# FrancescoI/torchrecsys

Hardware: AMD Instinct MI355X
Metric: training interactions/sec (pos+neg) (higher is better)
Workload: dtype f32; 1 GPU; c4 per-GPU shard: net_type='fm', 10M users x 1M items, 125M-interaction shard of 1B, dim=128, per-GPU batch 32768 (global 262144 at 8 GPUs); global_batch=32768, per_gpu_batch=32768, rng=device (Feistel epoch shuffle + Philox4x32-10 negative sampler)

## Files before the change

### torchrecsys_amd/csrc/api.cpp

```cpp
#include "trs_common.h"

#include <string.h>

static thread_local char g_err[512] = "";

void trs_set_error(const char* fmt, ...) {
  va_list ap;
  va_start(ap, fmt);
  vsnprintf(g_err, sizeof(g_err), fmt, ap);
  va_end(ap);
}

extern "C" const char* trs_last_error(void) { return g_err; }

#include <mutex>
#include <stdlib.h>

namespace {
struct Knob {
  const char* name;
  int64_t TrsTuning::*wide;
  int TrsTuning::*narrow;
  int64_t unset;
};
const Knob KNOBS[] = {
    {"GRID_CAP", &TrsTuning::grid_cap, nullptr, 256 * 16},
    {"PASS_GRID_CAP", &TrsTuning::pass_grid_cap, nullptr, 4096},
    {"PRESORT_GRID_CAP", &TrsTuning::presort_grid_cap, nullptr, 512},
    {"K1_ITERS", nullptr, &TrsTuning::k1_iters, 0},
    {"PASS_ITERS", nullptr, &TrsTuning::pass_iters, 0},
    {"PASS_NT", nullptr, &TrsTuning::pass_nt, -1},
    {"K1_NT", nullptr, &TrsTuning::k1_nt, -1},
    {"K1_WGS_PER_CU", nullptr, &TrsTuning::k1_wgs_per_cu, 2},
    {"GEMM32_NO_GLDS", nullptr, &TrsTuning::gemm32_no_glds, 0},
    {"GEMM16_TN_WIDE", nullptr, &TrsTuning::gemm16_tn_wide, -1},
    {"GEMM16_TILE", nullptr, &TrsTuning::gemm16_tile, 0},
    {"GEMM16_NO_GLDS", nullptr, &TrsTuning::gemm16_no_glds, 0},
    {"BN_FINAL_TWO_SWEEPS", nullptr, &TrsTuning::bn_final_two_sweeps, 0},
};
TrsTuning g_tuning;
std::once_flag g_tuning_once;
void knob_store(const Knob& k, int64_t v) {
  if (k.wide) g_tuning.*(k.wide) = v;
  else g_tuning.*(k.narrow) = (int)v;
}
}

TrsTuning& trs_tuning() {
  std::call_once(g_tuning_once, [] {
    for (const Knob& k : KNOBS) {
      char name[64];
      snprintf(name, sizeof(name), "TRS_%s", k.name);
      const char* e = getenv(name);
      knob_store(k, (e && *e) ? atoll(e) : k.unset);
    }
  });
  return g_tuning;
}

extern "C" int trs_tuning_set(const char* name, int64_t value, int32_t unset) {
  TRS_REQUIRE(name != nullptr, "trs_tuning_set: NULL name");
  (void)trs_tuning();
  for (const Knob& k : KNOBS)
    if (strcmp(k.name, name) == 0) {
      knob_store(k, unset ? k.unset : value);
      return TRS_OK;
    }
  trs_set_error("trs_tuning_set: unknown knob %s", name);
  return TRS_E_ARG;
}

extern "C" int trs_abi_version(void) { return TRS_ABI_VERSION; }

extern "C" int trs_check_device(void) {
  int dev = -1;
  if (hipGetDevice(&dev) != hipSuccess) {
    trs_set_error("trs_check_device: no HIP device");
    (void)hipGetLastError();
    return TRS_E_DEVICE;
  }
  hipDeviceProp_t p;
  if (hipGetDeviceProperties(&p, dev) != hipSuccess) {
    trs_set_error("trs_check_device: hipGetDeviceProperties failed");
    (void)hipGetLastError();
    return TRS_E_DEVICE;
  }
  if (strncmp(p.gcnArchName, "gfx950", 6) != 0) {
    trs_set_error("trs_check_device: device %d is %s, this library is built for gfx950 only", dev, p.gcnArchName);
    return TRS_E_DEVICE;
  }
  return TRS_OK;
}

extern "C" int trs_events_create(int32_t n, void** handles_out) {
  TRS_REQUIRE(n >= 0 && (n == 0 || handles_out), "trs_events_create: bad arguments");
  for (int32_t i = 0; i < n; ++i) {
    hipEvent_t e;
    if (hipEventCreate(&e) != hipSuccess) {
      trs_set_error("trs_events_create: hipEventCreate failed");
      (void)hipGetLastError();
      return TRS_E_LAUNCH;
    }
    handles_out[i] = (void*)e;
  }
  return TRS_OK;
}

extern "C" int trs_events_destroy(int32_t n, void** handles) {
  for (int32_t i = 0; i < n; ++i)
    if (handles && handles[i]) (void)hipEventDestroy((hipEvent_t)handles[i]);
  return TRS_OK;
}

extern "C" int trs_events_elapsed_ms(void* start, void* stop, float* ms_out) {
  TRS_REQUIRE(start && stop && ms_out, "trs_events_elapsed_ms: NULL argument");
  if (hipEventElapsedTime(ms_out, (hipEvent_t)start, (hipEvent_t)stop) != hipSuccess) {
    trs_set_error("trs_events_elapsed_ms: events not complete (synchronise the stream first)");
    (void)hipGetLastError();
    return TRS_E_LAUNCH;
  }
  return TRS_OK;
}
```

### torchrecsys_amd/csrc/presort.hip

```cpp
#include <cstring>

#include "score_kernels.h"
#include "opt_rows.h"

#ifndef K2_WAVES
#define K2_WAVES 4
#endif
namespace trs {

struct RefPayload {
  uint32_t tw;
};

struct EpochArgs {
  const int2* sui;
  const int32_t* neg_static;
  int64_t N;
  uint64_t shuffle_key;
  int hb;
  uint64_t sample_seed;
  int64_t first_pos;
  int64_t n_pos;
  int64_t batch;
  int64_t n_users, n_items;
  int item_bits;
  int32_t* user;
  int32_t* pos;
  int32_t* neg;
  void* keys;
  RefPayload* vals;
  int32_t* err;
  TrsSampler S;
};

template <typename KeyT, int SRC>
__global__ __launch_bounds__(TRS_BLOCK) void epoch_refs_kernel(const EpochArgs a) {
  const int64_t stride = (int64_t)gridDim.x * TRS_BLOCK;
  KeyT* keys = reinterpret_cast<KeyT*>(a.keys);
  for (int64_t q = (int64_t)blockIdx.x * TRS_BLOCK + threadIdx.x; q < a.n_pos; q += stride) {
    int64_t u, i, j;
    if (SRC != 0) {
      const int64_t p = trs_feistel_perm(a.first_pos + q, a.N * a.S.k_neg, a.shuffle_key, a.hb) % a.N;
      const int2 ui = a.sui[p];
      u = ui.x;
      i = ui.y;
      j = SRC == 2 ? (int64_t)a.neg_static[p]
                   : ((uint64_t)u < (uint64_t)a.n_users && (uint64_t)i < (uint64_t)a.n_items
                          ? trs_sample_neg_opt(a.sample_seed, (uint64_t)(a.first_pos + q), u, i, a.n_items, a.S)
                          : 0);
    } else {
      u = a.user[q];
      i = a.pos[q];
      j = a.neg[q];
    }
    bool ok = true;
    if ((uint64_t)u >= (uint64_t)a.n_users) { ok = false; u = 0; }
    if ((uint64_t)i >= (uint64_t)a.n_items) { ok = false; i = 0; }
    if ((uint64_t)j >= (uint64_t)a.n_items) { ok = false; j = 0; }
    if (!ok && a.err) atomicOr(a.err, 1);
    if (SRC != 0 || !ok) {
      a.user[q] = (int32_t)u;
      a.pos[q] = (int32_t)i;
      a.neg[q] = (int32_t)j;
    }
    if (keys) {
      keys[2 * q] = (KeyT)i;
      keys[2 * q + 1] = (KeyT)j;
    }
  }
}

struct FlagArgs {
  const int2* sui;
  const int32_t* neg_static;
  int64_t N;
  uint64_t shuffle_key;
  int hb;
  uint64_t sample_seed;
  int64_t first_pos, batch;
  int64_t n_users, n_items;
  int32_t *user, *pos, *neg;
  uint8_t* uflags;
  uint8_t* iflags;
  int32_t* err;
  int log2_bits;
  int item_hash, user_hash;
  int what_first, what_end;
  int32_t* nflag;
  int ord_off, ord_cap;
};

constexpr int FLAG_THREADS = 1024;

__device__ __forceinline__ uint32_t flag_bit(int32_t row, int hashed, int log2_bits) {
  return hashed ? ((uint32_t)row * 2654435761u) >> (32 - log2_bits) : (uint32_t)row;
}

constexpr int FLAG_U = 8;
constexpr int FLAG_ROUNDS = 8;
constexpr int FLAG_MAX_GROUPS = 4;

template <int NG>
__global__ __launch_bounds__(FLAG_THREADS) void batch_flags_kernel(const FlagArgs a) {
  extern __shared__ uint32_t bm[];
  const int words = 1 << (a.log2_bits - 5);
  const int64_t q0 = (int64_t)blockIdx.x * a.batch;
  const int B = (int)a.batch;
  const int lb = a.log2_bits;
  uint16_t* iflags16 = reinterpret_cast<uint16_t*>(a.iflags);
  constexpr int STEP = FLAG_THREADS * FLAG_U;
  uint64_t anyf[NG];
#pragma unroll
  for (int g = 0; g < NG; ++g) anyf[g] = 0;
  for (int what = a.what_first; what < a.what_end; ++what) {
    const int hashed = what == 0 ? a.item_hash : a.user_hash;
    const int32_t* ida = what == 0 ? a.pos : a.user;
    uint64_t lat0[NG], lat1[NG];
#pragma unroll
    for (int g = 0; g < NG; ++g) lat0[g] = lat1[g] = 0;
    for (int w = threadIdx.x; w < words; w += FLAG_THREADS) bm[w] = 0u;
    __syncthreads();
#pragma unroll
    for (int g = 0; g < NG; ++g) {
#pragma unroll 1
    for (int rr = 0; rr < FLAG_ROUNDS && (g * FLAG_ROUNDS + rr) * STEP < B; ++rr) {
      const int rd = g * FLAG_ROUNDS + rr;
      const int t0 = threadIdx.x + rd * STEP;
      uint32_t b0[FLAG_U], b1[FLAG_U];
#pragma unroll
      for (int k = 0; k < FLAG_U; ++k) {
        const int t = t0 + k * FLAG_THREADS;
        const int64_t q = q0 + (t < B ? t : 0);
        b0[k] = flag_bit(ida[q], hashed, lb);
        b1[k] = what == 0 ? flag_bit(a.neg[q], hashed, lb) : 0u;
      }
#pragma unroll
      for (int k = 0; k < FLAG_U; ++k) {
        if (t0 + k * FLAG_THREADS < B) {
          const uint32_t o0 = atomicOr(&bm[b0[k] >> 5], 1u << (b0[k] & 31));
          lat0[g] |= (uint64_t)((o0 >> (b0[k] & 31)) & 1u) << (rr * FLAG_U + k);
          if (what == 0) {
            const uint32_t o1 = atomicOr(&bm[b1[k] >> 5], 1u << (b1[k] & 31));
            lat1[g] |= (uint64_t)((o1 >> (b1[k] & 31)) & 1u) << (rr * FLAG_U + k);
          }
        }
      }
    }
    }
    __syncthreads();
    for (int w = threadIdx.x; w < words; w += FLAG_THREADS) bm[w] = 0u;
    __syncthreads();
#pragma unroll
    for (int g = 0; g < NG; ++g) {
      for (uint64_t m = lat0[g]; m; m &= m - 1) {
        const int bit = __ffsll((unsigned long long)m) - 1;
        const int64_t q = q0 + threadIdx.x + (int64_t)(g * FLAG_ROUNDS + bit / FLAG_U) * STEP + (bit % FLAG_U) * FLAG_THREADS;
        const uint32_t b = flag_bit(ida[q], hashed, lb);
        atomicOr(&bm[b >> 5], 1u << (b & 31));
      }
      for (uint64_t m = lat1[g]; m; m &= m - 1) {
        const int bit = __ffsll((unsigned long long)m) - 1;
        const int64_t q = q0 + threadIdx.x + (int64_t)(g * FLAG_ROUNDS + bit / FLAG_U) * STEP + (bit % FLAG_U) * FLAG_THREADS;
        const uint32_t b = flag_bit(a.neg[q], hashed, lb);
        atomicOr(&bm[b >> 5], 1u << (b & 31));
      }
    }
    __syncthreads();
#pragma unroll
    for (int g = 0; g < NG; ++g) {
#pragma unroll 1
    for (int rr = 0; rr < FLAG_ROUNDS && (g * FLAG_ROUNDS + rr) * STEP < B; ++rr) {
      const int t0 = threadIdx.x + (g * FLAG_ROUNDS + rr) * STEP;
      uint32_t b0[FLAG_U], b1[FLAG_U];
#pragma unroll
      for (int k = 0; k < FLAG_U; ++k) {
        const int t = t0 + k * FLAG_THREADS;
        const int64_t q = q0 + (t < B ? t : 0);
        b0[k] = flag_bit(ida[q], hashed, lb);
        b1[k] = what == 0 ? flag_bit(a.neg[q], hashed, lb) : 0u;
      }
#pragma unroll
      for (int k = 0; k < FLAG_U; ++k) {
        const int t = t0 + k * FLAG_THREADS;
        if (t < B) {
          const uint32_t s0 = (bm[b0[k] >> 5] >> (b0[k] & 31)) & 1u;
          const uint32_t s1 = what == 0 ? (bm[b1[k] >> 5] >> (b1[k] & 31)) & 1u : 0u;
          if (what == 0) iflags16[q0 + t] = (uint16_t)(s0 | (s1 << 8));
          else a.uflags[q0 + t] = (uint8_t)s0;
          anyf[g] |= (uint64_t)(s0 | s1) << (rr * FLAG_U + k);
        }
      }
    }
    }
    __syncthreads();
  }
  if (!a.nflag) return;
  {
    const int cells = (B + 63) >> 6;
    uint32_t* F = bm;
    uint32_t* holes = bm + a.ord_off;
    uint32_t* movers = holes + a.ord_cap;
    __shared__ uint32_t s_nf, s_flnf;
    const int lane = threadIdx.x & 63, wv = threadIdx.x >> 6;
    constexpr int NWV = FLAG_THREADS / 64;
#define TRS_FOR_MY_CELLS(BODY)                                                                     \
    _Pragma("unroll") for (int g = 0; g < NG; ++g) {                                                \
      _Pragma("unroll 1") for (int rr = 0; rr < FLAG_ROUNDS && (g * FLAG_ROUNDS + rr) * STEP < B; ++rr) { \
        _Pragma("unroll") for (int k = 0; k < FLAG_U; ++k) {                                        \
          const int j = (g * FLAG_ROUNDS + rr) * FLAG_U + k;                                       \
          const int c = wv + NWV * j;                                                              \
          const int t = c * 64 + lane;                                                             \
          const bool f = t < B && ((anyf[g] >> (rr * FLAG_U + k)) & 1ull) != 0;                    \
          const uint64_t bal = __ballot(f);                                                        \
          if (c < cells) { BODY }                                                                  \
        }                                                                                          \
      }                                                                                            \
    }
    TRS_FOR_MY_CELLS(if (lane == 0) F[c] = (uint32_t)__popcll((unsigned long long)bal);)
    __syncthreads();
    if (wv == 0) {
      const int per = (cells + 63) >> 6;
      uint32_t sum = 0;
      for (int i = 0; i < per; ++i) {
        const int c = lane * per + i;
        if (c < cells) sum += F[c];
      }
      uint32_t incl = sum;
#pragma unroll
      for (int off = 1; off < 64; off <<= 1) {
        const uint32_t v = __shfl_up(incl, off, 64);
        if (lane >= off) incl += v;
      }
      uint32_t run = incl - sum;
      for (int i = 0; i < per; ++i) {
        const int c = lane * per + i;
        if (c < cells) {
          const uint32_t v = F[c];
          F[c] = run;
          run += v;
        }
      }
      if (lane == 63) s_nf = s_flnf = incl;
    }
    __syncthreads();
    const int nf = (int)s_nf;
    TRS_FOR_MY_CELLS(
      const uint32_t fl = F[c] + (uint32_t)__popcll((unsigned long long)(bal & ((1ull << lane) - 1ull)));
      if (t == nf) s_flnf = fl;
      if (t < nf && !f && t - fl < (uint32_t)a.ord_cap) holes[t - fl] = (uint32_t)t;)
    __syncthreads();
    const uint32_t flnf = s_flnf;
    const int m = nf - (int)flnf;
    if (m > a.ord_cap) {
      if (threadIdx.x == 0) a.nflag[blockIdx.x] = B;
      return;
    }
    TRS_FOR_MY_CELLS(
      const uint32_t fl = F[c] + (uint32_t)__popcll((unsigned long long)(bal & ((1ull << lane) - 1ull)));
      if (t >= nf && f) movers[fl - flnf] = (uint32_t)t;)
#undef TRS_FOR_MY_CELLS
    __syncthreads();
    for (int k = threadIdx.x; k < m; k += FLAG_THREADS) {
      const int64_t x = q0 + holes[k], y = q0 + movers[k];
      const int32_t ux = a.user[x], px = a.pos[x], nx = a.neg[x], uy = a.user[y], py = a.pos[y], ny = a.neg[y];
      const uint8_t fux = a.uflags[x], fuy = a.uflags[y];
      const uint16_t fix = iflags16[x], fiy = iflags16[y];
// ... 660 lines not shown
  sorted_user_dup_update_body<KeyT, VEC, G, K, FULL>(a, blockIdx.x, gridDim.x);
}

template <int VEC, int G, int K, bool FULL, int OPT = OPT_SGD>
__global__ __launch_bounds__(TRS_BLOCK)
__attribute__((amdgpu_waves_per_eu(OPT == OPT_SGD && VEC == 4 && K == 1 && FULL ? K2_WAVES : 1)))
void sorted_updates_fused_kernel(const SortedArgs ia, const UserDupArgs ua,
                                                                        int n_user_blocks) {
  if ((int)blockIdx.x < n_user_blocks) {
    if (OPT == OPT_SGD && ua.ukeys == nullptr) flagged_user_update_body(ua, blockIdx.x, n_user_blocks);
    else sorted_user_dup_update_body<uint32_t, VEC, G, K, FULL, OPT>(ua, blockIdx.x, n_user_blocks);
  } else
    sorted_item_update_staged_body<uint32_t, VEC, G, K, FULL, OPT>(ia, (int)blockIdx.x - n_user_blocks,
                                                                   (int)gridDim.x - n_user_blocks);
}

static inline int presort_grid(int64_t n_pos) {
  const int64_t cap = n_pos <= ((int64_t)1 << 20) ? 4096 : trs_tuning().presort_grid_cap;
  int64_t g = (n_pos + TRS_BLOCK - 1) / TRS_BLOCK;
  return (int)(g < 1 ? 1 : (g > cap ? cap : g));
}

static int bits_for(int64_t n) {
  int b = 1;
  while (b < 63 && ((int64_t)1 << b) < n) ++b;
  return b;
}

template <int SRC>
static int launch_group(const int32_t* pos, const int32_t* neg, int64_t n_batches, int64_t batch, int64_t n_rows,
                        int pay_bits, uint32_t* keys_out, RefPayload* vals_out, hipStream_t s, const char* who) {
  const int refs_bits = bits_for((SRC == 2 ? 1 : 2) * batch);
  int bin_bits = 32 - pay_bits;
  if (bin_bits > GRP_MAX_BIN_BITS) bin_bits = GRP_MAX_BIN_BITS;
  if (bin_bits < GRP_MIN_BIN_BITS || ((int64_t)1 << refs_bits) / GRP_CAP + 2 > GRP_WMAX) {
    trs_set_error("%s: a batch of %lld positions is too long for the per-batch grouping (at most 2^21 references)", who,
                  (long long)batch);
    return TRS_E_ARG;
  }
  const size_t lds = (size_t)GRP_LDS_WORDS * 4;
  const dim3 gr((unsigned)n_batches), bl(GRP_THREADS);
#define TRS_GRP(BB)                                                                                                 \
  case BB: {                                                                                                        \
    static const int attr_done = [] {  \
      (void)hipFuncSetAttribute((const void*)batch_group_items_kernel<SRC, BB>, hipFuncAttributeMaxDynamicSharedMemorySize, \
                                GRP_LDS_WORDS * 4);                                                                  \
      return 1;                                                                                                     \
    }();                                                                                                            \
    (void)attr_done;                                                                                                \
    hipLaunchKernelGGL((batch_group_items_kernel<SRC, BB>), gr, bl, lds, s, pos, neg, batch, n_rows, pay_bits, keys_out, \
                       vals_out);                                                                                   \
    break;                                                                                                          \
  }
  switch (bin_bits) {
    TRS_GRP(14)
    TRS_GRP(13)
    TRS_GRP(12)
    TRS_GRP(11)
    TRS_GRP(10)
  }
#undef TRS_GRP
  TRS_CHECK_LAUNCH("batch_group_items_kernel");
  return TRS_OK;
}

}

using namespace trs;

extern "C" int trs_epoch_presort_sizes(int64_t n_batches, int64_t batch, int64_t n_items, int64_t* key_bytes_out,
                                       int64_t* keys_total_bytes_out, int64_t* vals_total_bytes_out,
                                       int64_t* temp_bytes_out) {
  TRS_REQUIRE(n_batches > 0 && batch > 0 && n_items > 0, "trs_epoch_presort_sizes: bad arguments");
  TRS_REQUIRE(key_bytes_out && keys_total_bytes_out && vals_total_bytes_out && temp_bytes_out,
              "trs_epoch_presort_sizes: NULL output");
  const int bits = bits_for(n_items);
  TRS_REQUIRE(bits <= 32 && 2 * n_batches * batch < ((int64_t)1 << 32), "trs_epoch_presort_sizes: slice too long");
  const int kb = 4;
  const size_t n = (size_t)(2 * n_batches * batch);
  const size_t temp = 0;
  *key_bytes_out = kb;
  *keys_total_bytes_out = 2 * (int64_t)n * kb;
  *vals_total_bytes_out = 2 * (int64_t)n * (int64_t)sizeof(RefPayload);
  *temp_bytes_out = (int64_t)temp + 256;
  return TRS_OK;
}

extern "C" int trs_epoch_presort(const int32_t* stream_ui_dev, const int32_t* neg_static_dev, int64_t N,
                                 uint64_t shuffle_key, uint64_t sample_seed, int64_t first_pos, int64_t n_batches,
                                 int64_t batch, int64_t n_users, int64_t n_items, int32_t* user_dev, int32_t* pos_dev,
                                 int32_t* neg_dev, void* keys_dev, void* vals_dev, void* temp_dev, int64_t temp_bytes,
                                 int32_t* err_flag_dev, void** sorted_keys_out, void** sorted_vals_out,
                                 uint8_t* item_dup_flags_out_dev, const trs_sampler* sampler, void* stream) {
  TRS_REQUIRE(n_batches > 0 && batch > 0 && n_users > 0 && n_items > 0, "trs_epoch_presort: bad sizes");
  TRS_TRY(trs_check_sampler("trs_epoch_presort", sampler));
  TRS_REQUIRE(user_dev && pos_dev && neg_dev && keys_dev && vals_dev && temp_dev, "trs_epoch_presort: NULL buffer");
  TRS_REQUIRE(sorted_keys_out && sorted_vals_out, "trs_epoch_presort: NULL output");
  const int64_t n_pos = n_batches * batch;
  int64_t kn = 1;
  if (stream_ui_dev) TRS_TRY(trs_check_slice("trs_epoch_presort", N, first_pos, n_pos, sampler, kn));
  EpochArgs a = {};
  a.S = trs_sampler_args(sampler);
  a.sui = (const int2*)stream_ui_dev;
  a.neg_static = neg_static_dev;
  a.N = N;
  a.shuffle_key = shuffle_key;
  a.hb = stream_ui_dev ? trs_feistel_half_bits(N * kn) : 0;
  a.sample_seed = sample_seed;
  a.first_pos = first_pos;
  a.n_pos = n_pos;
  a.batch = batch;
  a.n_users = n_users;
  a.n_items = n_items;
  a.item_bits = bits_for(n_items);
  a.user = user_dev;
  a.pos = pos_dev;
  a.neg = neg_dev;
  a.keys = keys_dev;
  a.vals = (RefPayload*)vals_dev;
  a.err = err_flag_dev;
  const int bits = a.item_bits;
  TRS_REQUIRE(bits <= 32 && 2 * n_pos < ((int64_t)1 << 32), "trs_epoch_presort: slice too long");
  const int src = !stream_ui_dev ? 0 : (neg_static_dev ? 2 : 1);
  hipStream_t s = (hipStream_t)stream;
  const dim3 gr(presort_grid(n_pos)), bl(TRS_BLOCK);
  const int pay_bits = bits_for(2 * batch);
  a.keys = nullptr;
  if (src == 0) hipLaunchKernelGGL((epoch_refs_kernel<uint32_t, 0>), gr, bl, 0, s, a);
  else if (src == 1) hipLaunchKernelGGL((epoch_refs_kernel<uint32_t, 1>), gr, bl, 0, s, a);
  else hipLaunchKernelGGL((epoch_refs_kernel<uint32_t, 2>), gr, bl, 0, s, a);
  TRS_CHECK_LAUNCH("epoch_refs_kernel");
  const size_t n = (size_t)(2 * n_pos);
  (void)temp_bytes;
  RefPayload* vin = (RefPayload*)vals_dev;
  RefPayload* vout = vin + n;
  uint32_t* kin = (uint32_t*)keys_dev;
  const int rc = launch_group<0>((const int32_t*)pos_dev, (const int32_t*)neg_dev, n_batches, batch, n_items, pay_bits,
                                 kin + n, vout, s, "trs_epoch_presort");
  if (rc) return rc;
  *sorted_keys_out = (void*)(kin + n);
  *sorted_vals_out = (void*)vout;
  if (item_dup_flags_out_dev) {
    (void)hipMemsetAsync(item_dup_flags_out_dev, 0, n, s);
    hipLaunchKernelGGL(item_flags_kernel, dim3(trs_grid((int64_t)n, TRS_BLOCK)), bl, 0, s, kin + n, vout, (int64_t)n,
                       2 * batch, item_dup_flags_out_dev);
    TRS_CHECK_LAUNCH("item_flags_kernel");
  }
  return TRS_OK;
}

static int launch_flags(const FlagArgs& a, int64_t n_batches, size_t lds, hipStream_t s) {
  const int64_t per_group = (int64_t)FLAG_THREADS * FLAG_U * FLAG_ROUNDS;
  const int ng = (int)((a.batch + per_group - 1) / per_group);
  const dim3 gr((unsigned)n_batches), bl(FLAG_THREADS);
#define TRS_FL(NG)                                                                                                   \
  {                                                                                                                  \
    static const int attr_done = [] {                    \
      (void)hipFuncSetAttribute((const void*)batch_flags_kernel<NG>, hipFuncAttributeMaxDynamicSharedMemorySize, 128 * 1024); \
      return 1;                                                                                                      \
    }();                                                                                                             \
    (void)attr_done;                                                                                                 \
    hipLaunchKernelGGL((batch_flags_kernel<NG>), gr, bl, lds, s, a);                                                  \
  }
  if (ng <= 1) TRS_FL(1) else if (ng == 2) TRS_FL(2) else TRS_FL(4)
#undef TRS_FL
  TRS_CHECK_LAUNCH("batch_flags_kernel");
  return TRS_OK;
}

extern "C" int trs_epoch_flags_ordered(const int32_t* stream_ui_dev, const int32_t* neg_static_dev, int64_t N,
                                       uint64_t shuffle_key, uint64_t sample_seed, int64_t first_pos, int64_t n_batches,
                                       int64_t batch, int64_t n_users, int64_t n_items, int32_t* user_dev,
                                       int32_t* pos_dev, int32_t* neg_dev, uint8_t* user_dup_flags_out_dev,
                                       uint8_t* item_dup_flags_out_dev, int32_t* n_flagged_out_dev,
                                       int32_t* err_flag_dev, const trs_sampler* sampler, void* stream);

extern "C" int trs_epoch_flags(const int32_t* stream_ui_dev, const int32_t* neg_static_dev, int64_t N,
                               uint64_t shuffle_key, uint64_t sample_seed, int64_t first_pos, int64_t n_batches,
                               int64_t batch, int64_t n_users, int64_t n_items, int32_t* user_dev, int32_t* pos_dev,
                               int32_t* neg_dev, uint8_t* user_dup_flags_out_dev, uint8_t* item_dup_flags_out_dev,
                               int32_t* err_flag_dev, const trs_sampler* sampler, void* stream) {
  return trs_epoch_flags_ordered(stream_ui_dev, neg_static_dev, N, shuffle_key, sample_seed, first_pos, n_batches, batch,
                                 n_users, n_items, user_dev, pos_dev, neg_dev, user_dup_flags_out_dev,
                                 item_dup_flags_out_dev, nullptr, err_flag_dev, sampler, stream);
}

extern "C" int trs_epoch_flags_ordered(const int32_t* stream_ui_dev, const int32_t* neg_static_dev, int64_t N,
                                       uint64_t shuffle_key, uint64_t sample_seed, int64_t first_pos, int64_t n_batches,
                                       int64_t batch, int64_t n_users, int64_t n_items, int32_t* user_dev,
                                       int32_t* pos_dev, int32_t* neg_dev, uint8_t* user_dup_flags_out_dev,
                                       uint8_t* item_dup_flags_out_dev, int32_t* n_flagged_out_dev,
                                       int32_t* err_flag_dev, const trs_sampler* sampler, void* stream) {
  TRS_TRY(trs_check_sampler("trs_epoch_flags", sampler));
  TRS_REQUIRE(batch <= (int64_t)FLAG_THREADS * FLAG_U * FLAG_ROUNDS * FLAG_MAX_GROUPS,
              "trs_epoch_flags: batch %lld exceeds %d (one workgroup per batch keeps a bit per reference in registers)",
              (long long)batch, FLAG_THREADS * FLAG_U * FLAG_ROUNDS * FLAG_MAX_GROUPS);
  TRS_REQUIRE(n_batches > 0 && batch > 0 && batch < ((int64_t)1 << 30) && n_users > 0 && n_items > 0 &&
                  n_users < ((int64_t)1 << 31) && n_items < ((int64_t)1 << 31), "trs_epoch_flags: bad sizes");
  TRS_REQUIRE(user_dev && pos_dev && neg_dev && user_dup_flags_out_dev && item_dup_flags_out_dev,
              "trs_epoch_flags: NULL buffer");
  int64_t kn = 1;
  if (stream_ui_dev) TRS_TRY(trs_check_slice("trs_epoch_flags", N, first_pos, n_batches * batch, sampler, kn));
  FlagArgs a = {};
  a.sui = (const int2*)stream_ui_dev;
  a.neg_static = neg_static_dev;
  a.N = N;
  a.shuffle_key = shuffle_key;
  a.hb = stream_ui_dev ? trs_feistel_half_bits(N) : 0;
  a.sample_seed = sample_seed;
  a.first_pos = first_pos;
  a.batch = batch;
  a.n_users = n_users;
  a.n_items = n_items;
  a.user = user_dev;
  a.pos = pos_dev;
  a.neg = neg_dev;
  a.uflags = user_dup_flags_out_dev;
  a.iflags = item_dup_flags_out_dev;
  a.err = err_flag_dev;
  const int64_t big = n_users > n_items ? n_users : n_items;
  int lb = 10;
  while (lb < 20 && ((int64_t)1 << lb) < big) ++lb;
  a.log2_bits = lb;
  a.item_hash = n_items > ((int64_t)1 << lb) ? 1 : 0;
  a.user_hash = n_users > ((int64_t)1 << lb) ? 1 : 0;
  a.what_first = 0;
  a.what_end = 2;
  size_t lds = ((size_t)1 << lb) / 8;
  if (n_flagged_out_dev) {
    a.nflag = n_flagged_out_dev;
    a.ord_off = (int)(((batch + 63) / 64 + 64) & ~(int64_t)63);
    const int64_t half = (batch + 1) / 2;
    a.ord_cap = (int)(half < 12288 ? (half < 64 ? 64 : half) : 12288);
    const size_t need = ((size_t)a.ord_off + 2 * (size_t)a.ord_cap) * 4;
    if (need > lds) lds = need;
  }
  int src = !stream_ui_dev ? 0 : (neg_static_dev ? 2 : 1);
  hipStream_t s = (hipStream_t)stream;
  if (src != 0) {
    EpochArgs e = {};
    e.sui = a.sui; e.neg_static = a.neg_static; e.N = a.N; e.shuffle_key = a.shuffle_key; e.hb = a.hb;
    e.sample_seed = a.sample_seed; e.first_pos = a.first_pos; e.n_pos = n_batches * batch; e.batch = batch;
    e.n_users = n_users; e.n_items = n_items; e.user = user_dev; e.pos = pos_dev; e.neg = neg_dev; e.keys = nullptr;
    e.err = err_flag_dev;
    e.S = trs_sampler_args(sampler);
    e.hb = trs_feistel_half_bits(N * kn);
    const dim3 ge(presort_grid(e.n_pos)), be(TRS_BLOCK);
    if (src == 1) hipLaunchKernelGGL((epoch_refs_kernel<uint32_t, 1>), ge, be, 0, s, e);
    else hipLaunchKernelGGL((epoch_refs_kernel<uint32_t, 2>), ge, be, 0, s, e);
    TRS_CHECK_LAUNCH("epoch_refs_kernel");
    src = 0;
  }
  (void)src;
  const int rcf = launch_flags(a, n_batches, lds, s);
  if (rcf) return rcf;
  TRS_CHECK_LAUNCH("batch_flags_kernel");
  return TRS_OK;
}

extern "C" int trs_epoch_user_flags(const int32_t* user_dev, int64_t n_batches, int64_t batch, int64_t n_users,
                                    uint8_t* flags_out_dev, void* stream) {
  TRS_REQUIRE(user_dev && flags_out_dev && n_batches > 0 && batch > 0 && n_users > 0 && n_users < ((int64_t)1 << 31),
              "trs_epoch_user_flags: bad arguments");
  TRS_REQUIRE(batch <= (int64_t)FLAG_THREADS * FLAG_U * FLAG_ROUNDS * FLAG_MAX_GROUPS,
              "trs_epoch_user_flags: batch %lld exceeds %d", (long long)batch,
              FLAG_THREADS * FLAG_U * FLAG_ROUNDS * FLAG_MAX_GROUPS);
  FlagArgs a = {};
  a.batch = batch;
  a.n_users = n_users;
  a.n_items = n_users;
  a.user = const_cast<int32_t*>(user_dev);
  a.pos = a.neg = a.user;
  a.uflags = flags_out_dev;
  int lb = 10;
  while (lb < 20 && ((int64_t)1 << lb) < n_users) ++lb;
  a.log2_bits = lb;
  a.user_hash = n_users > ((int64_t)1 << lb) ? 1 : 0;
  a.what_first = 1;
  a.what_end = 2;
  const int rcf = launch_flags(a, n_batches, ((size_t)1 << lb) / 8, (hipStream_t)stream);
  if (rcf) return rcf;
  TRS_CHECK_LAUNCH("batch_flags_kernel");
  return TRS_OK;
}

extern "C" int trs_epoch_user_dups_sizes(int64_t n_batches, int64_t batch, int64_t n_users, int64_t* ukeys_bytes_out,
                                         int64_t* uvals_bytes_out, int64_t* temp_bytes_out) {
  TRS_REQUIRE(n_batches > 0 && batch > 0 && n_users > 0 && ukeys_bytes_out && uvals_bytes_out && temp_bytes_out,
              "trs_epoch_user_dups_sizes: bad arguments");
  TRS_REQUIRE(n_batches * batch < ((int64_t)1 << 32), "trs_epoch_user_dups_sizes: slice too long");
  const int bits = bits_for(n_users);
  TRS_REQUIRE(bits <= 32, "trs_epoch_user_dups_sizes: user ids do not fit 32 bits");
  const int kb = 4;
  const size_t n = (size_t)(n_batches * batch);
  const size_t temp = 0;
  *ukeys_bytes_out = 2 * (int64_t)n * kb;
  *uvals_bytes_out = 2 * (int64_t)n * 4;
  *temp_bytes_out = (int64_t)temp + 256;
  return TRS_OK;
}

extern "C" int trs_epoch_user_dups(const int32_t* user_dev, int64_t n_batches, int64_t batch, int64_t n_users,
                                   void* ukeys_dev, void* uvals_dev, void* temp_dev, int64_t temp_bytes,
                                   uint8_t* flags_out_dev, void** sorted_ukeys_out, void** sorted_uvals_out,
                                   int32_t* ukey_bytes_out, void* stream) {
  TRS_REQUIRE(user_dev && ukeys_dev && uvals_dev && temp_dev && flags_out_dev, "trs_epoch_user_dups: NULL buffer");
  TRS_REQUIRE(n_batches > 0 && batch > 0 && n_users > 0 && n_batches * batch < ((int64_t)1 << 32),
              "trs_epoch_user_dups: bad sizes");
  const int64_t n_pos = n_batches * batch;
  const int user_bits = bits_for(n_users);
  TRS_REQUIRE(user_bits <= 32, "trs_epoch_user_dups: user ids do not fit 32 bits");
  hipStream_t s = (hipStream_t)stream;
  const dim3 gr(trs_grid(n_pos, TRS_BLOCK)), bl(TRS_BLOCK);
  (void)temp_bytes;
  uint32_t* vin = (uint32_t*)uvals_dev;
  uint32_t* kin = (uint32_t*)ukeys_dev;
  const int rc = launch_group<2>(user_dev, (const int32_t*)nullptr, n_batches, batch, n_users, bits_for(batch),
// ... 251 lines not shown
```

### torchrecsys_amd/csrc/trs_common.h

```cpp
#pragma once
#include <hip/hip_runtime.h>
#include <stdint.h>
#include <stdio.h>
#include <stdarg.h>
#include <stdlib.h>

#include "../../include/trs.h"

#define TRS_WAVE 64
#define TRS_BLOCK 256

void trs_set_error(const char* fmt, ...);

#define TRS_REQUIRE(cond, ...)        \
  do {                                \
    if (!(cond)) {                    \
      trs_set_error(__VA_ARGS__);     \
      return TRS_E_ARG;               \
    }                                 \
  } while (0)

#define TRS_TRY(expr)           \
  do {                          \
    const int rc__ = (expr);    \
    if (rc__) return rc__;      \
  } while (0)

#define TRS_CHECK_LAUNCH(name)                                           \
  do {                                                                     \
    hipError_t e__ = hipGetLastError();                                    \
    if (e__ != hipSuccess) {                                               \
      trs_set_error("%s: launch failed: %s", name, hipGetErrorString(e__)); \
      return TRS_E_LAUNCH;                                                 \
    }                                                                      \
  } while (0)

struct TrsTuning {
  int64_t grid_cap;
  int64_t pass_grid_cap;
  int64_t presort_grid_cap;
  int k1_iters;
  int pass_iters;
  int pass_nt;
  int k1_nt;
  int k1_wgs_per_cu;
  int gemm32_no_glds;
  int gemm16_tn_wide;
  int gemm16_tile;
  int gemm16_no_glds;
  int bn_final_two_sweeps;
};
TrsTuning& trs_tuning();

static inline int trs_grid(int64_t work_items, int items_per_block) {
  const int64_t cap = trs_tuning().grid_cap;
  int64_t g = (work_items + items_per_block - 1) / items_per_block;
  if (g < 1) g = 1;
  if (g > cap) g = cap;
  return (int)g;
}

__device__ __forceinline__ int64_t trs_ld_idx(const void* p, int idx_bytes, int64_t t) {
  return idx_bytes == 8 ? ((const int64_t*)p)[t] : (int64_t)((const int32_t*)p)[t];
}
__device__ __forceinline__ void trs_st_idx(void* p, int idx_bytes, int64_t t, int64_t v) {
  if (idx_bytes == 8)
    ((int64_t*)p)[t] = v;
  else
    ((int32_t*)p)[t] = (int32_t)v;
}

struct trs_u4 {
  uint32_t x, y, z, w;
};
__host__ __device__ __forceinline__ trs_u4 trs_philox4x32_10(uint64_t counter, uint64_t key) {
  uint32_t c0 = (uint32_t)counter, c1 = (uint32_t)(counter >> 32), c2 = 0u, c3 = 0u;
  uint32_t k0 = (uint32_t)key, k1 = (uint32_t)(key >> 32);
#pragma unroll
  for (int r = 0; r < 10; ++r) {
    uint64_t p0 = (uint64_t)0xD2511F53u * c0;
    uint64_t p1 = (uint64_t)0xCD9E8D57u * c2;
    uint32_t n0 = (uint32_t)(p1 >> 32) ^ c1 ^ k0;
    uint32_t n1 = (uint32_t)p1;
    uint32_t n2 = (uint32_t)(p0 >> 32) ^ c3 ^ k1;
    uint32_t n3 = (uint32_t)p0;
    c0 = n0; c1 = n1; c2 = n2; c3 = n3;
    k0 += 0x9E3779B9u;
    k1 += 0xBB67AE85u;
  }
  trs_u4 o = {c0, c1, c2, c3};
  return o;
}

__host__ __device__ __forceinline__ uint64_t trs_mulhi64(uint64_t a, uint64_t b) {
#ifdef __HIP_DEVICE_COMPILE__
  return __umul64hi(a, b);
#else
  return (uint64_t)(((unsigned __int128)a * (unsigned __int128)b) >> 64);
#endif
}

__host__ __device__ __forceinline__ int64_t trs_sample_one_neg(uint64_t seed, uint64_t ctr, int64_t pos,
                                                               int64_t n_items) {
  trs_u4 r = trs_philox4x32_10(ctr, seed);
  uint64_t x = ((uint64_t)r.y << 32) | (uint64_t)r.x;
  if (n_items <= 1) return 0;
  int64_t v = (int64_t)trs_mulhi64(x, (uint64_t)(n_items - 1));
  return v + (v >= pos ? 1 : 0);
}

__device__ __forceinline__ void trs_pair_loss(int kind, float sp, float sn, float& value, float& dneg) {
  if (kind == TRS_LOSS_BPR) {
    const float x = sn - sp;
    value = fmaxf(x, 0.f) + log1pf(expf(-fabsf(x)));
    dneg = 1.0f / (1.0f + expf(-x));
  } else {
    const float h = sn - sp + 1.0f;
    value = fmaxf(h, 0.f);
    dneg = h >= 0.f ? 1.f : 0.f;
  }
}

struct TrsSampler {
  int k_neg, popularity, max_tries;
  const int64_t* seen_off;
  const int32_t* seen_items;
  const int32_t* pop_items;
  int64_t pop_n;
  int64_t seen_users;
};
static inline TrsSampler trs_sampler_args(const trs_sampler* s) {
  TrsSampler r = {1, 0, 0, nullptr, nullptr, nullptr, 0, 0};
  if (s) {
    r.k_neg = s->k_neg < 1 ? 1 : s->k_neg;
    r.popularity = s->popularity;
    r.max_tries = s->max_tries < 1 ? 1 : s->max_tries;
    r.seen_off = s->seen_off;
    r.seen_items = s->seen_items;
    r.pop_items = s->pop_items;
    r.pop_n = s->pop_n;
    r.seen_users = s->seen_users;
  }
  return r;
}
constexpr uint64_t TRS_CANDIDATE_KEY_STEP = 0xD1B54A32D192ED03ull;

static inline int trs_check_sampler(const char* who, const trs_sampler* s) {
  TRS_REQUIRE(!s || (s->k_neg >= 1 && (!s->popularity || (s->pop_items && s->pop_n > 0)) &&
                     ((s->seen_off == nullptr) == (s->seen_items == nullptr))),
              "%s: bad sampler options", who);
  return TRS_OK;
}
static inline int trs_check_slice(const char* who, int64_t N, int64_t t0, int64_t B, const trs_sampler* s,
                                  int64_t& kn) {
  kn = s && s->k_neg > 1 ? s->k_neg : 1;
  TRS_REQUIRE(N > 0 && t0 >= 0 && B >= 0 && t0 + B <= N * kn, "%s: slice [%lld,%lld) outside [0,%lld)", who,
              (long long)t0, (long long)(t0 + B), (long long)(N * kn));
  return TRS_OK;
}
static inline int trs_check_net(const char* who, int net, const trs_tables* T) {
  TRS_REQUIRE(T != nullptr, "%s: tables is NULL", who);
  TRS_REQUIRE(net == TRS_NET_LINEAR || net == TRS_NET_FM, "%s: net must be TRS_NET_LINEAR or TRS_NET_FM", who);
  TRS_REQUIRE(T->M >= 0 && T->M <= TRS_MAX_META, "%s: M=%d outside 0..%d", who, T->M, TRS_MAX_META);
  return TRS_OK;
}
enum {
  TRS_SKIP_USER = 1,
  TRS_SKIP_USER_LIN = 2,
  TRS_SKIP_META_ROWS = 4,
};
static inline int trs_check_tables(const char* who, int net, const trs_tables* T, unsigned skip = 0,
                                   int64_t max_items = INT64_MAX) {
  TRS_TRY(trs_check_net(who, net, T));
  const bool user = !(skip & TRS_SKIP_USER);
  TRS_REQUIRE((!user || T->user) && T->item, "%s: user/item table is NULL", who);
  TRS_REQUIRE(!user || (skip & TRS_SKIP_USER_LIN) || T->user_lin, "%s: 1-wide user table (bias / linear term) is NULL",
              who);
  TRS_REQUIRE(T->item_lin, "%s: 1-wide item table (bias / linear term) is NULL", who);
  TRS_REQUIRE((!user || T->n_users > 0) && T->n_items > 0, "%s: empty user/item table", who);
  TRS_REQUIRE(T->n_items <= max_items, "%s: n_items=%lld above %lld", who, (long long)T->n_items,
              (long long)max_items);
  for (int m = 0; m < T->M; ++m) {
    TRS_REQUIRE(T->meta[m] && ((skip & TRS_SKIP_META_ROWS) || T->n_meta[m] > 0), "%s: metadata table %d is NULL/empty",
                who, m);
    if (net == TRS_NET_FM) TRS_REQUIRE(T->meta_lin[m], "%s: linear_metadata table %d is NULL", who, m);
  }
  return TRS_OK;
}

__device__ __forceinline__ bool trs_user_has_item(const TrsSampler& S, int64_t u, int64_t item) {
  if ((uint64_t)u >= (uint64_t)S.seen_users) return false;
  int64_t lo = S.seen_off[u], hi = S.seen_off[u + 1];
  while (lo < hi) {
    const int64_t mid = (lo + hi) >> 1;
    const int64_t v = S.seen_items[mid];
    if (v == item) return true;
    if (v < item) lo = mid + 1; else hi = mid;
  }
  return false;
}
__device__ __forceinline__ int64_t trs_sample_neg_opt(uint64_t seed, uint64_t ctr, int64_t u, int64_t pos,
                                                      int64_t n_items, const TrsSampler& S) {
  if (S.max_tries == 0) return trs_sample_one_neg(seed, ctr, pos, n_items);
// ... 90 lines not shown
```

Before: 1.997 billion interactions/s.

## Hold batch ids in registers across flag passes in batch_flags_kernel

```diff
diff --git a/torchrecsys_amd/csrc/api.cpp b/torchrecsys_amd/csrc/api.cpp
--- a/torchrecsys_amd/csrc/api.cpp
+++ b/torchrecsys_amd/csrc/api.cpp
@@ -37,6 +37,7 @@
     {"GEMM16_TILE", nullptr, &TrsTuning::gemm16_tile, 0},
     {"GEMM16_NO_GLDS", nullptr, &TrsTuning::gemm16_no_glds, 0},
     {"BN_FINAL_TWO_SWEEPS", nullptr, &TrsTuning::bn_final_two_sweeps, 0},
+    {"FLAGS_HELD", nullptr, &TrsTuning::flags_held, -1},
 };
 TrsTuning g_tuning;
 std::once_flag g_tuning_once;
diff --git a/torchrecsys_amd/csrc/presort.hip b/torchrecsys_amd/csrc/presort.hip
--- a/torchrecsys_amd/csrc/presort.hip
+++ b/torchrecsys_amd/csrc/presort.hip
@@ -100,9 +100,98 @@
 constexpr int FLAG_ROUNDS = 8;
 constexpr int FLAG_MAX_GROUPS = 4;
 
-template <int NG>
+constexpr int FLAG_HELD_ROUNDS = 4;
+constexpr int FLAG_HELD_N = FLAG_U * FLAG_HELD_ROUNDS;
+constexpr int FLAG_HELD_MAX = FLAG_THREADS * FLAG_HELD_N;
+constexpr uint32_t FLAG_HELD_MASK = (1u << 20) - 1u;
+
+__device__ __forceinline__ void flag_clear16(uint32_t* bm, int words) {
+  uint4* bm4 = reinterpret_cast<uint4*>(bm);
+  for (int w = threadIdx.x; w < (words >> 2); w += FLAG_THREADS) bm4[w] = make_uint4(0u, 0u, 0u, 0u);
+}
+
+__device__ __forceinline__ void flag_held_pin(uint64_t (&held)[FLAG_HELD_N], uint32_t& vm) {
+#pragma unroll
+  for (int j = 0; j < FLAG_HELD_N; ++j) asm volatile("" : "+v"(held[j]));
+  asm volatile("" : "+v"(vm));
+}
+
+__device__ __forceinline__ int flag_tid() {
+  int tid = threadIdx.x;
+  asm volatile("" : "+v"(tid));
+  return tid;
+}
+
+template <bool ITEMS>
+__device__ __forceinline__ void flags_held_pass(uint32_t* bm, int words, uint64_t (&held)[FLAG_HELD_N], uint32_t& vm,
+                                                int B, uint32_t& f0, uint32_t& f1) {
+  constexpr int STEP = FLAG_THREADS * FLAG_U;
+  uint32_t lat0 = 0, lat1 = 0;
+  f0 = f1 = 0;
+  flag_clear16(bm, words);
+  __syncthreads();
+  flag_held_pin(held, vm);
+#pragma unroll
+  for (int r = 0; r < FLAG_HELD_ROUNDS; ++r) {
+    if (r * STEP < B) {
+#pragma unroll
+      for (int k = 0; k < FLAG_U; ++k) {
+        const int j = r * FLAG_U + k;
+        const uint32_t v = (vm >> j) & 1u;
+        const uint32_t b0 = ITEMS ? (uint32_t)held[j] & FLAG_HELD_MASK : (uint32_t)(held[j] >> 40);
+        const uint32_t o0 = atomicOr(&bm[b0 >> 5], v << (b0 & 31));
+        lat0 |= ((o0 >> (b0 & 31)) & v) << j;
+        if (ITEMS) {
+          const uint32_t b1 = (uint32_t)(held[j] >> 20) & FLAG_HELD_MASK;
+          const uint32_t o1 = atomicOr(&bm[b1 >> 5], v << (b1 & 31));
+          lat1 |= ((o1 >> (b1 & 31)) & v) << j;
+        }
+      }
+    }
+  }
+  __syncthreads();
+  flag_clear16(bm, words);
+  __syncthreads();
+  flag_held_pin(held, vm);
+#pragma unroll
+  for (int r = 0; r < FLAG_HELD_ROUNDS; ++r) {
+    if (r * STEP < B) {
+#pragma unroll
+      for (int k = 0; k < FLAG_U; ++k) {
+        const int j = r * FLAG_U + k;
+        const uint32_t b0 = ITEMS ? (uint32_t)held[j] & FLAG_HELD_MASK : (uint32_t)(held[j] >> 40);
+        if ((lat0 >> j) & 1u) atomicOr(&bm[b0 >> 5], 1u << (b0 & 31));
+        if (ITEMS) {
+          const uint32_t b1 = (uint32_t)(held[j] >> 20) & FLAG_HELD_MASK;
+          if ((lat1 >> j) & 1u) atomicOr(&bm[b1 >> 5], 1u << (b1 & 31));
+        }
+      }
+    }
+  }
+  __syncthreads();
+  flag_held_pin(held, vm);
+#pragma unroll
+  for (int r = 0; r < FLAG_HELD_ROUNDS; ++r) {
+    if (r * STEP < B) {
+#pragma unroll
+      for (int k = 0; k < FLAG_U; ++k) {
+        const int j = r * FLAG_U + k;
+        const uint32_t v = (vm >> j) & 1u;
+        const uint32_t b0 = ITEMS ? (uint32_t)held[j] & FLAG_HELD_MASK : (uint32_t)(held[j] >> 40);
+        f0 |= ((bm[b0 >> 5] >> (b0 & 31)) & v) << j;
+        if (ITEMS) {
+          const uint32_t b1 = (uint32_t)(held[j] >> 20) & FLAG_HELD_MASK;
+          f1 |= ((bm[b1 >> 5] >> (b1 & 31)) & v) << j;
+        }
+      }
+    }
+  }
+  __syncthreads();
+}
+
+template <int NG, int HELD = 0>
 __global__ __launch_bounds__(FLAG_THREADS) void batch_flags_kernel(const FlagArgs a) {
-  extern __shared__ uint32_t bm[];
+  extern __shared__ __attribute__((aligned(16))) uint32_t bm[];
   const int words = 1 << (a.log2_bits - 5);
   const int64_t q0 = (int64_t)blockIdx.x * a.batch;
   const int B = (int)a.batch;
@@ -112,6 +201,51 @@
   uint64_t anyf[NG];
 #pragma unroll
   for (int g = 0; g < NG; ++g) anyf[g] = 0;
+  if constexpr (HELD != 0) {
+    static_assert(NG == 1 && FLAG_HELD_ROUNDS <= FLAG_ROUNDS, "the held triples' flags are bits 0-31 of anyf[0]");
+    uint64_t held[FLAG_HELD_N];
+    uint32_t vm = 0;
+    {
+      int32_t ru[FLAG_HELD_N], rp[FLAG_HELD_N], rn[FLAG_HELD_N];
+      const int tid = flag_tid();
+#pragma unroll
+      for (int j = 0; j < FLAG_HELD_N; ++j) {
+        const int t = tid + j * FLAG_THREADS;
+        const uint32_t off = 4u * (uint32_t)(t < B ? t : B - 1);
+        ru[j] = *reinterpret_cast<const int32_t*>(reinterpret_cast<const char*>(a.user + q0) + off);
+        rp[j] = HELD == 2 ? *reinterpret_cast<const int32_t*>(reinterpret_cast<const char*>(a.pos + q0) + off) : 0;
+        rn[j] = HELD == 2 ? *reinterpret_cast<const int32_t*>(reinterpret_cast<const char*>(a.neg + q0) + off) : 0;
+      }
+      const int tid2 = flag_tid();
+#pragma unroll
+      for (int j = 0; j < FLAG_HELD_N; ++j) vm |= (tid2 + j * FLAG_THREADS < B ? 1u : 0u) << j;
+#pragma unroll
+      for (int j = 0; j < FLAG_HELD_N; ++j)
+        held[j] = (uint64_t)(flag_bit(rp[j], a.item_hash, lb) & FLAG_HELD_MASK) |
+                  (uint64_t)(flag_bit(rn[j], a.item_hash, lb) & FLAG_HELD_MASK) << 20 |
+                  (uint64_t)(flag_bit(ru[j], a.user_hash, lb) & FLAG_HELD_MASK) << 40;
+    }
+    if constexpr (HELD == 2) {
+      uint32_t f0, f1;
+      flags_held_pass<true>(bm, words, held, vm, B, f0, f1);
+      asm volatile("" : "+v"(vm));
+      const int tid = flag_tid();
+#pragma unroll
+      for (int j = 0; j < FLAG_HELD_N; ++j)
+        if ((vm >> j) & 1u)
+          iflags16[q0 + tid + j * FLAG_THREADS] = (uint16_t)(((f0 >> j) & 1u) | (((f1 >> j) & 1u) << 8));
+      anyf[0] |= (uint64_t)(f0 | f1);
+    }
+    {
+      uint32_t f0, f1;
+      flags_held_pass<false>(bm, words, held, vm, B, f0, f1);
+      const int tid = flag_tid();
+#pragma unroll
+      for (int j = 0; j < FLAG_HELD_N; ++j)
+        if ((vm >> j) & 1u) a.uflags[q0 + tid + j * FLAG_THREADS] = (uint8_t)((f0 >> j) & 1u);
+      anyf[0] |= (uint64_t)f0;
+    }
+  } else
   for (int what = a.what_first; what < a.what_end; ++what) {
     const int hashed = what == 0 ? a.item_hash : a.user_hash;
     const int32_t* ida = what == 0 ? a.pos : a.user;
@@ -1078,17 +1212,20 @@
 static int launch_flags(const FlagArgs& a, int64_t n_batches, size_t lds, hipStream_t s) {
   const int64_t per_group = (int64_t)FLAG_THREADS * FLAG_U * FLAG_ROUNDS;
   const int ng = (int)((a.batch + per_group - 1) / per_group);
+  const int held = trs_tuning().flags_held != 0 && a.batch <= FLAG_HELD_MAX ? (a.what_first == 0 ? 2 : 1) : 0;
   const dim3 gr((unsigned)n_batches), bl(FLAG_THREADS);
-#define TRS_FL(NG)                                                                                                   \
+#define TRS_FL(NG, HELD)                                                                                             \
   {                                                                                                                  \
     static const int attr_done = [] {                    \
-      (void)hipFuncSetAttribute((const void*)batch_flags_kernel<NG>, hipFuncAttributeMaxDynamicSharedMemorySize, 128 * 1024); \
+      (void)hipFuncSetAttribute((const void*)batch_flags_kernel<NG, HELD>, hipFuncAttributeMaxDynamicSharedMemorySize, \
+                                128 * 1024);                                                                         \
       return 1;                                                                                                      \
     }();                                                                                                             \
     (void)attr_done;                                                                                                 \
-    hipLaunchKernelGGL((batch_flags_kernel<NG>), gr, bl, lds, s, a);                                                  \
-  }
-  if (ng <= 1) TRS_FL(1) else if (ng == 2) TRS_FL(2) else TRS_FL(4)
+    hipLaunchKernelGGL((batch_flags_kernel<NG, HELD>), gr, bl, lds, s, a);                                            \
+  }
+  if (held == 2) TRS_FL(1, 2) else if (held == 1) TRS_FL(1, 1)
+  else if (ng <= 1) TRS_FL(1, 0) else if (ng == 2) TRS_FL(2, 0) else TRS_FL(4, 0)
 #undef TRS_FL
   TRS_CHECK_LAUNCH("batch_flags_kernel");
   return TRS_OK;
diff --git a/torchrecsys_amd/csrc/trs_common.h b/torchrecsys_amd/csrc/trs_common.h
--- a/torchrecsys_amd/csrc/trs_common.h
+++ b/torchrecsys_amd/csrc/trs_common.h
@@ -49,6 +49,7 @@
   int gemm16_tile;
   int gemm16_no_glds;
   int bn_final_two_sweeps;
+  int flags_held;
 };
 TrsTuning& trs_tuning();
 
```

New measurement: 1.989 billion interactions/s. No clear change (-0.4%).
